# N-HANS/N-HANS

Measured on AMD Instinct MI355X. Metric: denoised audio seconds per second (16 kHz), whole job, higher is better.
Workload: dtype f16x3 (split hi+lo f16 operands, f32 accumulate); 1 GPU; 256 x 10 s 16 kHz synthetic mixture(s) per GPU, denoiser model, STFT+embed+mask+iSTFT end-to-end; clips_per_gpu=256, distinct_clips_per_gpu=256, frames_per_gpu=255488, weights=synthetic seed 7, parallelism=clip-sharded x1

## Files before the change

include/nhans_hip.h:

```cpp
#ifndef NHANS_HIP_H
#define NHANS_HIP_H

#include <stddef.h>
#include <stdint.h>

#ifdef __cplusplus
extern "C" {
#endif

#define NHANS_ABI_VERSION 5

#define NHANS_DENOISER 0
#define NHANS_SEPARATOR 1

#define NHANS_OK 0
#define NHANS_EINVAL (-1)
#define NHANS_EHIP (-2)
#define NHANS_ENOMEM (-3)
#define NHANS_ESHORT (-4)

#define NHANS_STATUS_SATURATED 1

#define NHANS_NUM_ACTIVATIONS 25

// ... 43 lines not shown
                        int nclips, const float* ctx_a_wav_dev, const int64_t* ctx_a_offsets_host,
                        const float* ctx_b_wav_dev, const int64_t* ctx_b_offsets_host,
                        float* denoised_wav_dev, float* mixed_wav_dev, float* logmag_out_dev,
                        float* phase_out_dev, float* logits_out_dev, float* emb_out_dev, void* stream);

int nhans_debug_block_output(nhans_ctx* ctx, const float* logmag_dev, const int64_t* frame_offsets_host,
                             int nclips, const float* emb_a_dev, const float* emb_b_dev,
                             int64_t frame0, int nframes, int block, float* out_dev, void* stream);

int nhans_debug_activation(nhans_ctx* ctx, const float* logmag_dev, const int64_t* frame_offsets_host,
                           int nclips, const float* emb_a_dev, const float* emb_b_dev,
                           int64_t frame0, int nframes, int index, float* out_dev, void* stream);
int nhans_debug_tower_activation(nhans_ctx* ctx, const float* ctx_logmag_dev, int n, int index, float* out_dev,
                                 void* stream);

int nhans_take_status(nhans_ctx* ctx, int* flags_out, void* stream);

int nhans_debug_launch_probe(size_t dynamic_lds_bytes, void* stream);

int nhans_debug_mfma_ceiling(double seconds, void* stream, double* sustained_tflops, double* first_tflops,
                             int* launches);

int nhans_debug_row_classes(int H, int KH, int stride, int pt, int* out, int cap);

uint32_t nhans_crc32c(uint32_t crc, const void* data_host, size_t nbytes);

typedef struct nhans_online nhans_online;

int nhans_online_open(nhans_ctx* ctx, int nstreams, const float* ctx_a_wav_dev, const int64_t* ctx_a_offsets_host,
                      const float* ctx_b_wav_dev, const int64_t* ctx_b_offsets_host, int want_mixed, void* stream,
                      nhans_online** out);

int nhans_online_open_slots(nhans_ctx* ctx, int nslots, int want_mixed, void* stream, nhans_online** out);

int nhans_online_restart(nhans_online* obj, int slot);

int nhans_online_set_context(nhans_online* obj, int slot, const float* ctx_a_wav_dev, int64_t na,
                             const float* ctx_b_wav_dev, int64_t nb, void* stream, int64_t* first_frame_out);

int nhans_online_set_embeddings(nhans_online* obj, int slot, const float* emb_a_dev, const float* emb_b_dev,
                                void* stream, int64_t* first_frame_out);


int nhans_online_push(nhans_online* obj, const float* in_dev, const int64_t* in_offsets_host, const int* end_host,
                      float* den_out_dev, float* mixed_out_dev, const int64_t* out_offsets_host,
                      int64_t* out_counts_host, void* stream);
// ... 106 lines not shown
```

n-hans_amd/csrc/conv_epilogue.h:

```cpp
#pragma once
#include "nhans_kernels.h"
#include <cstddef>

namespace nhans {

typedef float f32x16 __attribute__((ext_vector_type(16)));
typedef float f32x4 __attribute__((ext_vector_type(4)));
typedef _Float16 f16x8 __attribute__((ext_vector_type(8)));
typedef _Float16 f16x4 __attribute__((ext_vector_type(4)));

template <int I, int NM, int ND> __device__ __forceinline__ void pin_reads_between_mfmas() {
    if constexpr (I < ND) {
        __builtin_amdgcn_sched_group_barrier(0x008, (I + 1) * NM / ND - I * NM / ND, 0);
        __builtin_amdgcn_sched_group_barrier(0x100, 1, 0);
        pin_reads_between_mfmas<I + 1, NM, ND>();
    }
}

template <int I, int NM, int ND> __device__ __forceinline__ void pin_reads_front_loaded() {
    if constexpr (I < ND) {
        __builtin_amdgcn_sched_group_barrier(0x008, 1, 0);
        __builtin_amdgcn_sched_group_barrier(0x100, 1, 0);
        pin_reads_front_loaded<I + 1, NM, ND>();
    } else if constexpr (NM > ND) {
// ... 31 lines not shown
    else asm("v_fma_mix_f32 %0, %1, 1.0, %2 op_sel:[1,0,1] op_sel_hi:[1,0,1]" : "=v"(d) : "v"(hi_pair), "v"(lo_pair));
    return d;
}

__device__ __forceinline__ float split_load(const float* base, size_t row_floats, int n) {
    const _Float16* p = reinterpret_cast<const _Float16*>(base + row_floats) + (n >> 5) * 64 + (n & 31);
    return (float)p[0] + (float)p[32];
}

template <typename T> __device__ __forceinline__ T conv_karg(size_t offset) {
    typedef const __attribute__((address_space(4))) char* kptr;
    return *reinterpret_cast<const __attribute__((address_space(4))) T*>((kptr)__builtin_amdgcn_kernarg_segment_ptr() + offset);
}
#define CONV_KARG(FIELD) ::nhans::conv_karg<decltype(::nhans::ConvArgs::FIELD)>(offsetof(::nhans::ConvArgs, FIELD))

template <int BMROWS, int BNCOLS> constexpr size_t conv_epilogue_lds_bytes() {
    return (size_t)BMROWS * (BNCOLS + 4) * sizeof(float) + (size_t)BMROWS * sizeof(int4);
}

struct EpiTile {
    int m0;
    int tw, th;
    int b, r0, c0;
    __device__ __forceinline__ int operator()(int p, const ConvArgs& a) const {
        if (tw <= 0) {
            const int m = m0 + p;
            return m < a.M ? m : -1;
        }
        const int r = p / tw, c = p - r * tw;
        if (r >= th || r0 + r >= a.Ho || c0 + c >= a.Wo) return -1;
        return (b * a.Ho + r0 + r) * a.Wo + c0 + c;
    }
};

template <int PREC, int IDM, int OUTS, int PP, int PASSES, int LDC>
__device__ __forceinline__ void conv_epilogue_sweep(const ConvArgs& a, const float* ct, const int4* rowinfo,
                                                    int prow, int c4, int n) {
    constexpr int GP = PASSES < 8 ? PASSES : 8;
    static_assert(PASSES % GP == 0, "pass grouping");
    const int f_tf = a.tf ? 1 : 0;
    const float* __restrict__ cbp = a.cb;
    const float* __restrict__ tfp = a.tf ? a.tf : a.zero;
    f32x4 wsv = {1.f, 1.f, 1.f, 1.f}, idwv = {0.f, 0.f, 0.f, 0.f};
    if constexpr (PREC == 1) wsv = *reinterpret_cast<const f32x4*>(a.ws + n) * CONV_KARG(in_scale);
    if constexpr (IDM != 0) idwv = *reinterpret_cast<const f32x4*>(a.idw + n) * CONV_KARG(id_scale);
    const int hoff = (n >> 5) * 64 + (n & 31);
    const float lo_clamp = a.relu ? 0.f : -3.0e38f;
    const float osc = CONV_KARG(out_scale), slim = CONV_KARG(sat_limit);
    bool sat = false;
#pragma unroll 1
// ... 156 lines not shown
        }
    };

    Epi8Raw<IDM> ra[GP], rb[GP];
    issue(0, ra);
#pragma unroll
    for (int g = 0; g < NG; g += 2) {
        if (g + 1 < NG) issue(g + 1, rb);
        finish(ra);
        if (kDev && es && g == 0) {
            asm volatile("s_waitcnt lgkmcnt(0)" ::: "memory");
            es[2] = (long long)__builtin_amdgcn_s_memtime();
        }
        if (g + 2 < NG) issue(g + 2, ra);
        if (g + 1 < NG) finish(rb);
    }
    int* const satp = CONV_KARG(sat);
    if (sat && satp) atomicOr(satp, kSatActivation);
}

template <int TM, int TN, int PREC, int NTHREADS, int BMROWS, int BNCOLS>
__device__ __forceinline__ void conv_epilogue(const ConvArgs& a, f32x16 (&acc)[TM][TN], float* smem, EpiTile tile,
                                              int row_base, int col_base, int n_tile0, int tid, int lane,
                                              long long* es = nullptr ) {
    constexpr int LDC = BNCOLS + 4;
    constexpr int C4 = BNCOLS / 4;
    constexpr int PP = NTHREADS / C4;
    constexpr int PASSES = BMROWS / PP;
    float* ct = smem;
    int4* rowinfo = reinterpret_cast<int4*>(smem + BMROWS * LDC);

#pragma unroll
    for (int i = 0; i < TM; ++i)
#pragma unroll
        for (int j = 0; j < TN; ++j)
#pragma unroll
            for (int g = 0; g < 4; ++g) {
                const f32x4 v = {acc[i][j][4 * g], acc[i][j][4 * g + 1], acc[i][j][4 * g + 2], acc[i][j][4 * g + 3]};
                *reinterpret_cast<f32x4*>(ct + (row_base + i * 32 + (lane & 31)) * LDC + col_base + j * 32 + 8 * g +
                                          4 * (lane >> 5)) = v;
            }
    if (tid < BMROWS) {
        const int mz = tile(tid, a);
        const int m = mz < 0 ? (tile.tw > 0 ? tile(0, a) : a.M - 1) : mz;
        const uint32_t b = fd_div((uint32_t)m, a.fdHoWo);
        const uint32_t rem = (uint32_t)m - b * a.fdHoWo.d;
        const uint32_t ho = fd_div(rem, a.fdWo);
        const uint32_t wo = rem - ho * a.fdWo.d;
        const int clip = a.img_clip ? a.img_clip[b] : 0;
        const uint32_t hov = ho + (uint32_t)a.oh0;
        const int remv = (int)(hov * a.fdWo.d + wo);
        const int mv = mz < 0 ? mz : (int)(b * (uint32_t)a.Ho_full * a.fdWo.d) + remv;
        int ids;
        if (a.id_mode == 2 && a.id_win.t) {
            const int h = (int)hov * a.idsh;
            ids = win_row_ok(a.id_win, (int)b, h) ? win_row(a.id_win, (int)b, h) * a.idW + (int)wo * a.idsw : kNoRow;
        } else {
            ids = (int)((b * a.idH + hov * a.idsh) * a.idW + wo * a.idsw);
        }
        rowinfo[tid] = make_int4(clip * a.cb_stride, remv * a.N, mv, ids);
    }
    if (kDev && es) { asm volatile("s_waitcnt lgkmcnt(0)" ::: "memory"); es[0] = (long long)__builtin_amdgcn_s_memtime(); }
    __syncthreads();
    if (kDev && es) es[1] = (long long)__builtin_amdgcn_s_memtime();

    const int c4 = tid % C4, prow = tid / C4;
    const int n = n_tile0 + c4 * 4;
    const int f_tf = a.tf ? 1 : 0;
    const bool id_split = a.id_mode == 1 && a.id_split;
    const float* __restrict__ cbp = a.cb;
    const float* __restrict__ tfp = a.tf ? a.tf : a.zero;
    const bool vec = (a.Nreal == a.N) && !a.aux && (a.out_split || (a.ldo & 3) == 0) &&
                     (a.id_mode != 1 || id_split || (a.id_ld & 3) == 0);
// ... 55 lines not shown
```

n-hans_amd/csrc/conv_igemm_halo.hip:

```cpp
#include "conv_epilogue.h"
#include <cstdlib>

namespace nhans {

namespace {
constexpr int NCW = 8;
constexpr int NPW = 4;

template <int HBM_> struct HaloShape {
    static constexpr int HBM = HBM_;
    static constexpr int HR = HBM_ == 512 ? 544 : 320;
    static constexpr int BST = HBM_ == 512 ? 3 : 4;
    static constexpr int WN = HBM_ == 512 ? 1 : 2;
    static constexpr int NAP = HR * 8 / (NPW * 64);
};

template <int N> __device__ __forceinline__ void halo_wait_vmcnt() {
    asm volatile("s_waitcnt vmcnt(%0)" ::"n"(N) : "memory");
}
}

template <int BN, int PREC, int HBM_ = 256, int DBG = 0, int ABL = 0, int PWM = 0>
__global__ void __launch_bounds__((NCW + NPW) * 64) conv_igemm_halo(const ConvArgs a) {
    using SH = HaloShape<HBM_>;
    constexpr int HBM = SH::HBM, HR = SH::HR, BST = SH::BST, WN = SH::WN, NAP = SH::NAP;
    constexpr int PFD = BST - 1;
    constexpr int TM = 2;
    constexpr int TN = BN / (32 * WN);
    static_assert(HBM == (NCW / WN) * TM * 32 && BN == WN * TN * 32, "wave grid");
    static_assert(!PWM || (HBM == 256 && BST == 4), "pointwise mode: 256-pixel tiles, four weight stages");
    constexpr int A_BUF = (PWM ? HBM : HR) * 32;
    constexpr int NABUF = PWM ? 3 : 2;
    constexpr int NAPW = PWM ? HBM * 8 / (NPW * 64) : NAP;
    constexpr int B_STAGE = 32 * BN;
    constexpr int B_BASE = NABUF * A_BUF;
    constexpr int GBP = B_STAGE / 4 / (NPW * 64);
    extern __shared__ __attribute__((aligned(16))) float smem[];

    const int tid = threadIdx.x, lane = tid & 63;
    const int wave = __builtin_amdgcn_readfirstlane(tid >> 6);
    long long dbg_entry = 0;
    if constexpr (DBG) dbg_entry = (long long)__builtin_amdgcn_s_memtime();

    const int ntn = a.N / BN;
    int L;
    {
        const int nblk = gridDim.x, bid = blockIdx.x;
        const int q = nblk >> 3, r = nblk & 7, xcd = bid & 7, idx = bid >> 3;
        L = (xcd < r ? xcd * (q + 1) : r * (q + 1) + (xcd - r) * q) + idx;
    }
    const int mt = L / ntn, nt = L - mt * ntn;
    const int m0 = mt * HBM;
    const int nt0 = nt * (BN / 32);

    const int Wo = (int)a.fdWo.d;
    const int R0 = (int)fd_div((uint32_t)m0, a.fdWo);
    const int w0 = m0 - R0 * Wo;

    const int nseg = a.nseg;
    const int KW0 = a.seg[0].KW, KH0 = a.seg[0].KH, CC0 = a.seg[0].C >> 5;
    const int KH1 = nseg > 1 ? a.seg[1].KH : 0, CC1 = nseg > 1 ? (a.seg[1].C >> 5) : 0;
    const int nsup0 = KH0 * CC0 * (PWM ? KW0 : 1);
    const int nsup = nsup0 + KH1 * CC1;
    const int ntap0 = PWM ? nsup0 : nsup0 * KW0;
    const int total = ntap0 + KH1 * CC1;

    int segC = 0, kwC = 0, bufC = 0, supC = 0;
#define NH_NEXT_TAP()                                                                              \
    if constexpr (PWM) {                                                                           \
        bufC = bufC == NABUF - 1 ? 0 : bufC + 1;                                                   \
    } else if (++kwC >= (segC ? 1 : KW0)) {                                                        \
        kwC = 0;                                                                                   \
        bufC ^= 1;                                                                                 \
        if (++supC == nsup0) segC = 1;                                                             \
    }

    if (wave >= NCW) {
        const int pw = wave - NCW, ptid = tid - NCW * 64;
        if constexpr (!(ABL & 64)) __builtin_amdgcn_s_setprio(3);
        const int slot = lane & 7;
        const int nrows_all = a.M / Wo;
        const size_t bstride = (size_t)(a.N / 32) * 1024;
        constexpr unsigned kOob = 0x80000000u;
        const int b0 = (int)fd_div((uint32_t)m0, a.fdHoWo);
        int poff[NAPW], hov[NAPW], wiv[PWM ? NAPW : 1];
        int sH = 0, sW = 0, sC = 0;
        __amdgpu_buffer_rsrc_t srsrc;
#define NH_MAP_SEGMENT(S)                                                                          \
    {                                                                                              \
        const ConvSeg& g = a.seg[S];                                                               \
        sH = g.H; sW = g.W; sC = g.C;                                                              \
        {                                                                                          \
            const size_t fb_ = (size_t)g.H * g.W * g.C * 4;                                        \
            const size_t left_ = (size_t)(a.M / (a.Ho * Wo) - b0) * fb_;                           \
            srsrc = __builtin_amdgcn_make_buffer_rsrc(const_cast<float*>(g.src) + (size_t)b0 * (fb_ / 4), 0, \
                                                      (int)(left_ < 0x7FFFFFFFu ? left_ : 0x7FFFFFFFu), 0x00020000); \
        }                                                                                          \
        _Pragma("unroll") for (int d = 0; d < NAPW; ++d) {                                         \
            const int j = d * 32 + pw * 8 + (lane >> 3);                                           \
            const int sp = (slot ^ ((j >> 1) & 7)) * 4;                                            \
            int Rg, wi;                                                                            \
            bool ok;                                                                               \
            if (!PWM && g.KW > 1) {                                                                \
                const int n0 = Wo - w0 + g.KW - 1;                                                 \
                int i = 0, cj = w0 + j;                                                            \
                if (j >= n0) {                                                                     \
                    const int jj = j - n0;                                                         \
                    const int q = (int)fd_div((uint32_t)jj, a.fdWP);                               \
                    i = 1 + q;                                                                     \
                    cj = jj - q * (int)a.fdWP.d;                                                   \
                }                                                                                  \
                wi = cj - g.pl;                                                                    \
                Rg = R0 + i;                                                                       \
                ok = Rg < nrows_all && (unsigned)wi < (unsigned)g.W;                               \
            } else {                                                                               \
                const int m = m0 + j;                                                              \
                ok = j < HBM && m < a.M;                                                           \
                Rg = (int)fd_div((uint32_t)(ok ? m : 0), a.fdWo);                                  \
                wi = ((ok ? m : 0) - Rg * Wo) * g.sw - g.pl;                                       \
            }                                                                                      \
            if (!ok) { Rg = 0; wi = 0; }                                                           \
            const int b = (int)fd_div((uint32_t)(Rg * Wo), a.fdHoWo);                              \
            const int hi0 = (Rg - b * a.Ho) * g.sh - g.pt;                                         \
            poff[d] = ((((b - b0) * g.H + hi0) * g.W + wi) * g.C + sp) * 4;      \
            hov[d] = ok ? hi0 : -(1 << 28);                                                        \
            if constexpr (PWM) wiv[d] = wi;               \
        }                                                                                          \
    }
#define NH_GLDS(SRC, DST)                                                                          \
    __builtin_amdgcn_global_load_lds((const __attribute__((address_space(1))) void*)(SRC),        \
                                     (__attribute__((address_space(3))) void*)(DST), 16, 0, 0);

        int segA = 0, khA = 0, ccA = 0, supA = 0, kwA = 0;
#define NH_ISSUE_A(BUF)                                                                            \
    {                                                                                              \
        const int khoff_ = (khA * sW + (PWM ? kwA : 0)) * sC + ccA * 32;                           \
        const bool live_ = supA < nsup;                                                            \
        float* sa_ = smem + (BUF) * A_BUF + pw * 8 * 32;                                           \
        _Pragma("unroll") for (int d = 0; d < NAPW; ++d) {                                         \
            bool in_ = !(ABL & 1) && live_ && (unsigned)(hov[d] + khA) < (unsigned)sH;             \
            if constexpr (PWM) in_ = in_ && (unsigned)(wiv[d] + kwA) < (unsigned)sW;               \
            if constexpr (!(ABL & 2))                                                              \
                __builtin_amdgcn_raw_ptr_buffer_load_lds(srsrc, (__attribute__((address_space(3))) void*)(sa_ + d * 32 * 32), 16, \
                                                         in_ ? (unsigned)(poff[d] + khoff_ * 4) : kOob, 0, 0, 0); \
        }                                                                                          \
        ++supA;                                                                                    \
        if (PWM && ++kwA < KW0) {                  \
        } else if (kwA = 0, ++khA >= (segA ? KH1 : KH0)) {  \
            khA = 0;                                                                               \
            if (++ccA >= (segA ? CC1 : CC0)) {                                                     \
                ccA = 0;                                                                           \
                if (segA == 0 && nseg > 1) {                                                       \
                    segA = 1;                                                                      \
                    NH_MAP_SEGMENT(1)                                                              \
                }                                                                                  \
            }                                                                                      \
        }                                                                                          \
    }
        int tapB = 0;
        const __amdgpu_buffer_rsrc_t wr0 = __builtin_amdgcn_make_buffer_rsrc(const_cast<float*>(a.seg[0].wpk) + (size_t)nt0 * 1024, 0, 0x7FFFFFFF, 0x00020000);
        const __amdgpu_buffer_rsrc_t wr1 = __builtin_amdgcn_make_buffer_rsrc(const_cast<float*>(nseg > 1 ? a.seg[1].wpk : a.seg[0].wpk) + (size_t)nt0 * 1024, 0, 0x7FFFFFFF, 0x00020000);
        const unsigned wvo = (unsigned)ptid * 16u;
        const int bstride_b = (int)(bstride * 4);
        int wper = KH0 * KW0, wskip = (a.seg[0].KHfull - KH0) * KW0, wrun = 0;
        int wtap = a.seg[0].kh0 * KW0 - 1, wseg = 0;
#define NH_ISSUE_B(ST)                                                                             \
    {                                                                                              \
        if (tapB < total && !(ABL & 4)) {                                                          \
            if (tapB == ntap0) {                                                                   \
                wseg = 1; wtap = a.seg[1].kh0 * a.seg[1].KW; wrun = 1;                             \
                wper = KH1 * a.seg[1].KW; wskip = (a.seg[1].KHfull - KH1) * a.seg[1].KW;           \
            } else {                                                                               \
                if (wrun == wper) { wrun = 0; wtap += wskip; }                                     \
                ++wtap; ++wrun;                                                                    \
            }                                                                                      \
        }                                                                                          \
        ++tapB;                                                                                    \
        float* sb_ = smem + B_BASE + (ST) * B_STAGE;                                               \
        const int so_ = (ABL & 4) ? 0 : wtap * bstride_b;                                          \
        _Pragma("unroll") for (int j = 0; j < GBP; ++j)                                            \
            if constexpr (!(ABL & 8))                                                              \
                __builtin_amdgcn_raw_ptr_buffer_load_lds((wseg || (ABL & 4)) ? wr1 : wr0,          \
                    (__attribute__((address_space(3))) void*)(sb_ + (j * (NPW * 64) + pw * 64) * 4), 16, wvo, so_ + j * (NPW * 64) * 16, 0, 0); \
    }

        NH_MAP_SEGMENT(0)
        NH_ISSUE_A(0)
        NH_ISSUE_B(0)
// ... 162 lines not shown
            }
            acc[0][0][0] += k_;
        }
        __builtin_amdgcn_sched_barrier(0);
    }
    asm volatile("s_waitcnt lgkmcnt(0)" ::: "memory");
    __builtin_amdgcn_s_barrier();
    if constexpr (DBG) {
        if (a.dbg && lane == 0) {
            long long* d = a.dbg + ((size_t)blockIdx.x * (NCW + NPW) + wave) * 4;
            d[0] = (long long)__builtin_amdgcn_s_memtime() - dbg_t0; d[1] = dbg_t0 - dbg_entry; d[2] = 0; d[3] = dbg_bar;
        }
    }
#undef NH_READ_HALF
#undef NH_MFMA_HALF
#undef NH_NEXT_TAP
#undef NH_PIN_INTERLEAVE

    long long dbg_epi = 0;
    long long es[3] = {0, 0, 0};
    if constexpr (DBG) dbg_epi = (long long)__builtin_amdgcn_s_memtime();
    static_assert(conv_epilogue_lds_bytes<HBM, BN>() <= (size_t)(NABUF * A_BUF + BST * B_STAGE) * sizeof(float), "epilogue LDS");
    conv_epilogue<TM, TN, PREC, NCW * 64, HBM, BN>(a, acc, smem, EpiTile{m0, 0, 0, 0, 0, 0}, wm * 64, wn * TN * 32, nt * BN, tid, lane,
                                                   DBG ? es : nullptr);
    if constexpr (DBG) {
        const long long t_issued = (long long)__builtin_amdgcn_s_memtime();
        asm volatile("s_waitcnt vmcnt(0)" ::: "memory");
        if (a.dbg && lane == 0) {
            const long long t_end = (long long)__builtin_amdgcn_s_memtime();
            a.dbg[((size_t)blockIdx.x * (NCW + NPW) + wave) * 4 + 2] = t_end - dbg_epi;
            long long* e = a.dbg + (size_t)(4 << 20) + ((size_t)blockIdx.x * (NCW + NPW) + wave) * 8;
            e[0] = es[0] - dbg_epi; e[1] = es[1] - dbg_epi; e[2] = es[2] - dbg_epi; e[3] = t_issued - dbg_epi; e[4] = t_end - dbg_epi;
        }
    }
}

template <int BN, int PREC, int HBM_ = 256, int DBG = 0, int ABL = 0, int PWM = 0> static void launch_halo_t(const ConvArgs& a, hipStream_t s) {
    using SH = HaloShape<HBM_>;
    constexpr size_t lds = (size_t)((PWM ? 3 * SH::HBM : 2 * SH::HR) * 32 + SH::BST * 32 * BN) * sizeof(float);
    static_assert(lds <= 160 * 1024, "LDS of a gfx950 CU");
    static unsigned long long attr_devices = 0;
    set_max_dynamic_lds(reinterpret_cast<const void*>(&conv_igemm_halo<BN, PREC, HBM_, DBG, ABL, PWM>), lds, &attr_devices, "conv_igemm_halo");
    const int mtiles = (a.M + SH::HBM - 1) / SH::HBM;
    const int grid = mtiles * (a.N / BN);
    NHANS_LAUNCH("conv_igemm_halo", (conv_igemm_halo<BN, PREC, HBM_, DBG, ABL, PWM>), dim3(grid), dim3((NCW + NPW) * 64), lds, s, a);
}

static int halo_tile_pixels(const ConvArgs& a) { return (a.N % 128 != 0 && a.halo64_tile512) ? 512 : 256; }

bool conv_igemm_halo_eligible(const ConvArgs& a) {
    const ConvSeg& g = a.seg[0];
    if (g.KW < 3 || g.sw != 1 || a.Wo != g.W || g.pl < 0 || g.pl >= g.KW) return false;
    if (a.nseg > 1 && a.seg[1].KW != 1) return false;
    if (a.nseg > 2 || a.M % a.Wo != 0) return false;
    for (int i = 0; i < a.nseg; ++i) {
        const ConvSeg& q = a.seg[i];
        const double elems = (double)(a.M / (a.Ho * a.Wo)) * q.H * q.W * q.C;
        if (elems + 65536.0 >= 2147483648.0) return false;
    }
    const int hbm = halo_tile_pixels(a);
    const int nrows = (a.Wo - 1 + hbm - 1) / a.Wo + 1;
    return hbm + (g.KW - 1) * nrows <= (hbm == 512 ? HaloShape<512>::HR : HaloShape<256>::HR);
}

bool conv_igemm_halo_pw_eligible(const ConvArgs& a) {
    const ConvSeg& g = a.seg[0];
    if (a.nseg != 1 || a.N % 128 != 0 || a.kgroup != 0 || g.C % 32 != 0) return false;
// ... 61 lines not shown
```

n-hans_amd/csrc/host_ctx.hip:

```cpp
#include "host_internal.h"

namespace {

thread_local std::string g_err;

constexpr uint32_t kBlobVersion = 2;
struct BlobHeader {
    char magic[8];
    uint32_t version;
    uint32_t n_entries;
    uint64_t total_bytes;
};
struct BlobEntry {
    char name[48];
    uint64_t offset;
    uint64_t nfloats;
};

std::vector<BlockGeo> tower_geometry() {
    const int kh[4] = {8, 8, 4, 4}, kw[4] = {4, 4, 4, 4}, sh[4] = {3, 3, 1, 1}, sw[4] = {2, 2, 1, 2};
    const int co[4] = {64, 128, 256, 512};
    std::vector<BlockGeo> v;
    int h = kCtxFrames, w = kBins, c = 1;
    for (int i = 0; i < 4; ++i) {
// ... 343 lines not shown
    }
    else if (k == "conv_variant") {
        if (value < -1 || value > 2) return fail(NHANS_EINVAL, "conv_variant must be -1 (auto), 0, 1 or 2");
        c->conv_variant = (int)value;
    }
    else if (k == "calibrate") {
        if (value < 0 || value > 3) return fail(NHANS_EINVAL, "calibrate must be 1 (start), 0 (stop, set), 2 (stop, raise only) or 3 (stop, discard)");
        int rc = check_ctx(c); if (rc) return rc;
        if (value == 1) {
            HIP_TRY(hipDeviceSynchronize());
            HIP_TRY(hipMemset(c->amax_dev, 0, kNumAct * sizeof(unsigned)));
            c->calibrating = true;
        } else {
            if (!c->calibrating) return fail(NHANS_EINVAL, "calibrate: no bracket is open");
            if (value == 3) { c->calibrating = false; return NHANS_OK; }
            return finish_calibration(c, value == 2);
        }
    }
    else if (k == "winograd") c->wino = value != 0;
    else if (k == "winograd_f32_tensors") c->wino_f32 = (value == 2 || value == 3) ? (int)value : value != 0;
    else if (k == "split_k") c->split_k = value != 0;
    else if (k == "stream_1x1") c->stream_1x1 = value != 0;
    else if (k == "row_split") {
        if (value < 0 || value > 2) return fail(NHANS_EINVAL, "row_split must be 0, 1 or 2 (2: every conv that can be split, a measurement value)");
        c->row_split = (int)value;
    }
    else if (k == "precision") {
        if (value != 0 && value != 1) return fail(NHANS_EINVAL, "precision must be 0 (f32) or 1 (f16x3)");
        if (value == 1 && !c->A("head.dense.wpk_h"))
            return fail(NHANS_EINVAL, "the folded blob carries no split-f16 weights");
        c->prec = (int)value;
    }
    else return fail(NHANS_EINVAL, "unknown option " + k);
    return NHANS_OK;
}

int nhans_set_activation_exponents(nhans_ctx* c, const int* e, int n) {
    if (!c || !e || n != kNumAct) return fail(NHANS_EINVAL, "activation exponents: need NHANS_NUM_ACTIVATIONS values");
    for (int i = 0; i < n; ++i)
        if (e[i] < -60 || e[i] > 60) return fail(NHANS_EINVAL, "activation exponent outside [-60, 60]");
    std::copy(e, e + n, c->act_exp);
    tie_exponents(c);
    return NHANS_OK;
}

int nhans_get_activation_exponents(nhans_ctx* c, int* e_out, int n) {
    if (!c || !e_out || n != kNumAct) return fail(NHANS_EINVAL, "activation exponents: need NHANS_NUM_ACTIVATIONS values");
// ... 105 lines not shown
```

n-hans_amd/csrc/host_internal.h:

```cpp
#pragma once
#include "../../include/nhans_hip.h"
#include "nhans_kernels.h"

#include <algorithm>
#include <cmath>
#include <cstdio>
#include <cstdlib>
#include <cstring>
#include <limits>
#include <map>
#include <string>
#include <vector>

using namespace nhans;

#pragma GCC visibility push(hidden)

int fail(int code, const std::string& msg);

#define HIP_TRY(expr)                                                                          \
    do {                                                                                       \
        hipError_t e_ = (expr);                                                                \
        if (e_ != hipSuccess)                                                                  \
            return fail(NHANS_EHIP, std::string(#expr) + ": " + hipGetErrorString(e_));        \
// ... 18 lines not shown
#pragma GCC visibility pop

struct StackPlan {
    bool wino[8][3] = {};
};

struct nhans_ctx {
    int kind = 0, device = 0;
    StackPlan last_plan;
    float* blob_dev = nullptr;
    size_t blob_bytes = 0;
    std::map<std::string, const float*> arr;
    std::map<std::string, size_t> arr_n;
    std::vector<BlockGeo> tower, stack;
    int cond_cols = 0;
    std::vector<int> cond_off;
    char* ws = nullptr;
    size_t ws_bytes = 0, ws_top = 0;
    float* kscratch = nullptr;
    size_t kscratch_bytes = 0;
    static constexpr size_t kscratch_cap = (size_t)384 << 20;
    bool kscratch_failed = false;
    int stream_1x1 = 1;
    int row_split = 1;
    int split_k = 1;
    int* kcounter = nullptr;
    int kcounter_n = 1024;
    int64_t frames_per_chunk = 3776;
    int contexts_per_chunk = 64;
    int lookahead = kCenter;
    char* pin = nullptr;
    size_t pin_bytes = (size_t)16 << 20, pin_top = 0;
    bool profile = false;
    std::map<std::string, ProfEntry> prof;
    std::vector<hipEvent_t> event_pool;

    int prec = 0;
    int conv_variant = -1;
    int epi8 = 1;
    int ilv = 1;
    int wino = 1;
    int wino_f32 = 1;
    long long* dbg = nullptr;
    int* status_dev = nullptr;
    std::map<std::pair<int, int>, float*> rs_tab;
    int act_exp[kNumAct] = {};
    float act_amax[kNumAct] = {};
// ... 221 lines not shown
```

n-hans_amd/csrc/host_net.hip:

```cpp
#include "host_internal.h"

namespace {

void same_pad(int n, int k, int s, int* out, int* before) {
    *out = (n + s - 1) / s;
    int total = std::max((*out - 1) * s + k - n, 0);
    *before = total / 2;
}

void fill_epilogue_defaults(nhans_ctx* c, ConvArgs& a) {
    a.zero = c->A("zero");
    a.sat = c->status_dev;
    a.img_clip = nullptr; a.tf = nullptr; a.tt = nullptr; a.ff = nullptr; a.id_mode = 0; a.id = nullptr; a.id_ld = 0;
    a.idw = nullptr; a.idH = a.idW = 0; a.idsh = a.idsw = 1; a.relu = 1; a.aux = nullptr; a.aux_ld = 0;
    a.cb_stride = 0;
    a.prec = c->prec; a.out_split = c->prec; a.id_split = 0; a.ws = nullptr;
    a.in_scale = a.id_scale = a.out_scale = 1.f;
    a.sat_limit = kSatLimitF16;
    a.variant = c->conv_variant >= 0 ? c->conv_variant : (c->prec == 1 ? 2 : 0);
    a.dbg = kDev ? c->dbg : nullptr;
    a.epi8 = c->epi8;
    a.ilv = c->ilv;
    a.wino = c->wino; a.wino_u = nullptr; a.wino_ws = nullptr;
    a.kscratch = c->kscratch; a.kscratch_bytes = c->kscratch_bytes; a.kcounter = c->kcounter; a.kcounter_n = c->kcounter_n; a.kgroup = 0;
// ... 19 lines not shown
}

const char* run_conv(nhans_ctx* c, const ConvArgs& a0, hipStream_t s) {
    ConvArgs a = a0;
    if (kDev) {
        static const bool no_tf = [] { const char* e = getenv("NHANS_ABLATE_TF"); return e && atoi(e) != 0; }();
        if (no_tf) { a.tf = nullptr; a.tt = nullptr; a.ff = nullptr; }
    }
    if (a.kgroup < 0) {
        const size_t need = c->split_k ? conv_splitk_scratch_bytes(a) : 0;
        if (need > c->kscratch_bytes && need <= nhans_ctx::kscratch_cap && !c->kscratch_failed) {
            if (c->kscratch) { (void)hipFree(c->kscratch); c->kscratch = nullptr; c->kscratch_bytes = 0; }
            const size_t want = std::min(nhans_ctx::kscratch_cap, std::max(need, (size_t)32 << 20));
            if (hipMalloc(reinterpret_cast<void**>(&c->kscratch), want) == hipSuccess) c->kscratch_bytes = want;
            else { (void)hipGetLastError(); c->kscratch = nullptr; c->kscratch_failed = true; }
        }
        a.kscratch = c->split_k ? c->kscratch : nullptr;
        a.kscratch_bytes = c->kscratch_bytes;
    }
    Prof p(c, s, nullptr);
    const char* name = "conv_igemm";
    double mfma = 0;
    double fl = launch_conv_igemm(a, s, &name, &mfma);
    if (a.Ho_full != a.Ho) {
        double kfull = 0;
        for (int i = 0; i < a.nseg; ++i) kfull += (double)a.seg[i].KHfull * a.seg[i].KW * a.seg[i].C;
        fl = 2.0 * (double)a.M * kfull * (double)a.Nreal;
    }
    p.done(fl, 0, name, mfma);
    return name;
}

struct RowClass { int oh0, rows, kh0, kh; };

int row_classes(int H, int KH, int s, int pt, RowClass* out, int cap) {
    const int Ho = (H + s - 1) / s;
    int n = 0;
    for (int ho = 0; ho < Ho; ++ho) {
        const int hi0 = ho * s - pt;
        const int lo = std::max(0, -hi0), hi = std::min(KH, H - hi0);
        if (hi <= lo) return 0;
        if (n && out[n - 1].kh0 == lo && out[n - 1].kh == hi - lo) { ++out[n - 1].rows; continue; }
        if (n == cap) return -1;
        out[n++] = RowClass{ho, 1, lo, hi - lo};
    }
    return n;
}

bool row_split_pays(const ConvSeg& g, const RowClass* rc, int n) {
    int applied = 0, rows = 0;
    for (int i = 0; i < n; ++i) { applied += rc[i].rows * rc[i].kh; rows += rc[i].rows; }
    return 100 * (rows * g.KH - applied) >= 7 * rows * g.KH;
}

constexpr int kMaxRowClasses = 8;
bool halo_family(ConvArgs a) {
    if (a.variant < 2 || a.kgroup != 0 || a.N % 128 != 0 || a.in_f32 || conv_wino_eligible(a)) return false;
    a.halo64_tile512 = 0;
    return conv_igemm_halo_eligible(a) || conv_igemm_halo_pw_eligible(a);
}
bool run_conv_row_classes(nhans_ctx* c, const ConvArgs& a, hipStream_t s) {
    const ConvSeg& g = a.seg[0];
    if (!c->row_split || a.prec != 1 || a.Ho_full != a.Ho || a.M % (a.Ho * a.Wo) != 0 || !halo_family(a)) return false;
    if (a.nseg > 1 && a.seg[1].KH != 1) return false;
    RowClass rc[kMaxRowClasses];
    const int n = row_classes(g.H, g.KH, g.sh, g.pt, rc, kMaxRowClasses);
    if (n < 2 || (g.H + g.sh - 1) / g.sh != a.Ho) return false;
    if (c->row_split == 1 && !row_split_pays(g, rc, n)) return false;
    const int B = a.M / (a.Ho * a.Wo);
    ConvArgs q[kMaxRowClasses];
    for (int i = 0; i < n; ++i) {
        q[i] = a;
        q[i].Ho = rc[i].rows; q[i].M = B * rc[i].rows * a.Wo; q[i].oh0 = rc[i].oh0; q[i].Ho_full = a.Ho;
        q[i].fdHoWo = make_fastdiv((uint32_t)(rc[i].rows * a.Wo));
        ConvSeg& h = q[i].seg[0];
        h.KH = rc[i].kh; h.kh0 = rc[i].kh0; h.KHfull = g.KH; h.pt = g.pt - rc[i].kh0 - rc[i].oh0 * g.sh;
        h.nchunks = h.KH * h.KW * h.C / 32;
        if (a.nseg > 1) {
            ConvSeg& t = q[i].seg[1];
            if ((rc[i].oh0 + rc[i].rows - 1) * t.sh - t.pt >= t.H || rc[i].oh0 * t.sh - t.pt < 0) return false;
            t.pt -= rc[i].oh0 * t.sh;
        }
        q[i].wino_u = nullptr; q[i].wino_ws = nullptr;
        if (!halo_family(q[i])) return false;
    }
    for (int i = 0; i < n && !launch_error_pending(); ++i)
        if (std::strncmp(run_conv(c, q[i], s), "conv_igemm_halo", 15) != 0)
            note_refusal("row-class conv launch on a kernel that does not walk filter-row classes");
    return true;
}

bool wino_form(const ConvArgs& a) { return a.variant >= 2 && a.kgroup >= 0 && conv_wino_eligible(a); }
float sat_limit_for(const StackPlan& p, int b, int cv) { return b >= 0 && b < 8 && p.wino[b][cv] ? kSatLimitWinoInput : kSatLimitF16; }

bool stored_f32(const nhans_ctx* c, const StackPlan& p, int b, int cv) {
    if (c->prec != 1 || !c->wino_f32 || b < 0 || b > 7) return false;
    if (c->wino_f32 == 2) return b < 4 && !(b == 3 && cv == 1);
    if (c->wino_f32 == 3) return b == 1 && cv == 1;
    if (cv == 0) return p.wino[b][2] && (b == 0 || p.wino[b][1]);
    if (b == 7) return false;
    const BlockGeo& nx = c->stack[b + 1];
    return p.wino[b][2] && p.wino[b + 1][1] && nx.cin == nx.cout && p.wino[b + 1][2];
}

void tap(nhans_ctx* c, int idx, const float* buf, size_t words, int chan, hipStream_t s, bool f32_layout = false) {
    if (c->calibrating) launch_absmax(buf, words, c->prec && !f32_layout, c->up(idx), c->amax_dev + idx, s);
    if (c->cap_idx != idx) return;
// ... 500 lines not shown
    rc = h2d(c, sb.foff_dev, foff, (nclips + 1) * sizeof(int64_t), s); if (rc) return rc;
    launch_frame_index(sb.foff_dev, nclips, total, c->lookahead, sb.f_clip, sb.f_t, sb.f_T, s);
    launch_cond(ea, eb, nclips, c->A("cond.w"), c->A("cond.base"), c->cond_cols, sb.cb_all, s);
    const float* res = run_stack_chunk(c, logmag, nullptr, sb, frame0, nframes, block + 1, s);
    size_t per;
    if (block == 8) per = (size_t)26 * 512;
    else per = (size_t)c->stack[block].hout * c->stack[block].wout * c->stack[block].cout;
    if (c->prec && block < 8 && stored_f32(c, c->last_plan, block, 1)) launch_scale_copy(res, per * nframes, c->up(SA(block, 1)), out, s);
    else if (c->prec) launch_unsplit(res, (int64_t)nframes * (int64_t)(per / (block == 8 ? 512 : c->stack[block].cout)),
                                block == 8 ? 512 : c->stack[block].cout, c->up(block == 8 ? kActHead : SA(block, 1)), out, s);
    else HIP_TRY(hipMemcpyAsync(out, res, per * nframes * 4, hipMemcpyDeviceToDevice, s));
    return NHANS_OK;
}

int nhans_debug_row_classes(int H, int KH, int stride, int pt, int* out, int cap) {
    if (H < 1 || KH < 1 || stride < 1 || pt < 0 || cap < 0 || (cap && !out)) return fail(NHANS_EINVAL, "row classes: bad argument");
    std::vector<RowClass> rc((size_t)(H + stride - 1) / stride);
    const int n = row_classes(H, KH, stride, pt, rc.data(), (int)rc.size());
    if (n > cap) return fail(NHANS_EINVAL, "row classes: " + std::to_string(n) + " classes, room for " + std::to_string(cap));
    for (int i = 0; i < n; ++i) { out[4 * i] = rc[i].oh0; out[4 * i + 1] = rc[i].rows; out[4 * i + 2] = rc[i].kh0; out[4 * i + 3] = rc[i].kh; }
    return n;
}

int nhans_debug_block_output(nhans_ctx* c, const float* logmag, const int64_t* foff, int nclips, const float* ea,
                             const float* eb, int64_t frame0, int nframes, int block, float* out, void* stream) {
    Call call(c, stream);
    if (call.rc) return call.rc;
    return call.finish(debug_block_output_body(c, logmag, foff, nclips, ea, eb, frame0, nframes, block, out, stream));
}

static int debug_activation_body(nhans_ctx* c, const float* logmag, const int64_t* foff, int nclips, const float* ea,
                                 const float* eb, int64_t frame0, int nframes, int index, float* out, void* stream) {
    int rc = NHANS_OK;
    if (!logmag || !foff || !ea || !eb || !out || nclips < 1 || nframes < 1) return fail(NHANS_EINVAL, "bad argument");
    if (index < SA(0, 0) || index >= kNumAct)
        return fail(NHANS_EINVAL, "activation index outside the stack's 8 .. " + std::to_string(kNumAct - 1) + " (tower tensors: nhans_debug_tower_activation)");
    hipStream_t s = static_cast<hipStream_t>(stream);
    const int64_t total = foff[nclips];
    if (frame0 < 0 || frame0 + nframes > total) return fail(NHANS_EINVAL, "frame range outside batch");
    const int64_t wf = std::min<int64_t>(c->frames_per_chunk, nframes);
    rc = ws_reserve(c, stack_ws_bytes(c, total, nclips, wf)); if (rc) return rc;
    StackBufs sb;
    stack_take(c, total, nclips, wf, &sb);
    rc = h2d(c, sb.foff_dev, foff, (nclips + 1) * sizeof(int64_t), s); if (rc) return rc;
    launch_frame_index(sb.foff_dev, nclips, total, c->lookahead, sb.f_clip, sb.f_t, sb.f_T, s);
    launch_cond(ea, eb, nclips, c->A("cond.w"), c->A("cond.base"), c->cond_cols, sb.cb_all, s);
// ... 69 lines not shown
```

n-hans_amd/csrc/nhans_kernels.h:

```cpp
#pragma once
#include <hip/hip_runtime.h>
#include <stdint.h>

#include <tuple>
#include <utility>
#include <vector>

namespace nhans {

constexpr int kWin = 400, kHop = 160, kBins = 201, kMixWin = 35, kCtxFrames = 200, kEmb = 512;
constexpr int kCenter = kMixWin / 2;
constexpr int64_t kMaxFramesPerChunk = ((int64_t)1 << 31) / ((int64_t)kMixWin * kBins * 64);

#ifdef NHANS_DEV
constexpr bool kDev = true;
int dev_ablate();
#else
constexpr bool kDev = false;
constexpr int dev_ablate() { return 0; }
#endif

void note_launch(const char* kernel, hipError_t launch_rc);
bool launch_error_pending();
void note_refusal(const char* what);
// ... 36 lines not shown
struct WinRows {
    const int* t;
    const int* T;
    int row0, pad;
    const int* rb;
};
constexpr int kNoRow = -2147483647 - 1;
__device__ __forceinline__ bool win_row_ok(const WinRows& w, int b, int h) {
    return (unsigned)(w.t[b] + h - w.pad) < (unsigned)w.T[b];
}
__device__ __forceinline__ int win_row(const WinRows& w, int b, int h) {
    return (w.rb ? w.rb[b] : w.row0 + b) + h;
}

struct ConvSeg {
    const float* src;
    const float* wpk;
    int H, W, C;
    int KH, KW, sh, sw, pt, pl;
    int nchunks;
    int kh0, KHfull;
};

struct ConvArgs {
    ConvSeg seg[2];
    int nseg;
    int Ho, Wo;
    int M;
    int oh0, Ho_full;
    int N;
    int Nreal;
    int ldo;
    float* out;
    const float* cb;
    int cb_stride;
    const int* img_clip;
    const float* tf;
    const float* tt;
    const float* ff;
    int id_mode;
    const float* id;
    int id_ld;
    const float* idw;
    int idH, idW, idsh, idsw;
    WinRows id_win;
    int relu;
    float* aux;
    int aux_ld;
    const float* zero;
    int prec;
    int out_split;
    int id_split;
// ... 163 lines not shown
```

n-hans_amd/hip.py:

```python
import ctypes
import json
import os
import sys

_HERE = os.path.dirname(os.path.abspath(__file__))
LIB_PATH = os.environ.get("NHANS_LIB") or os.path.join(_HERE, "csrc", "libnhans_hip.so")

DENOISER, SEPARATOR = 0, 1
KIND_CODE = {"denoiser": DENOISER, "separator": SEPARATOR}

_int, _i64, _dbl, _vp = ctypes.c_int, ctypes.c_int64, ctypes.c_double, ctypes.c_void_p
_size, _str = ctypes.c_size_t, ctypes.c_char_p
_ip, _i64p, _vpp = ctypes.POINTER(_int), ctypes.POINTER(_i64), ctypes.POINTER(_vp)
_fp, _dp = ctypes.POINTER(ctypes.c_float), ctypes.POINTER(_dbl)
SIGNATURES = {
    "nhans_abi_version": (_int, []),
    "nhans_last_error": (_str, []),
    "nhans_num_frames": (_i64, [_i64]),
    "nhans_create": (_int, [_int, _vp, _size, _int, _vpp]),
    "nhans_create_ex": (_int, [_int, _vp, _size, _int, _ip, _int, _vpp]),
    "nhans_destroy": (None, [_vp]),
    "nhans_set_option": (_int, [_vp, _str, _i64]),
    "nhans_set_activation_exponents": (_int, [_vp, _ip, _int]),
    "nhans_get_activation_exponents": (_int, [_vp, _ip, _int]),
    "nhans_get_activation_amax": (_int, [_vp, _fp, _int]),
    "nhans_workspace_bytes": (_size, [_vp, _i64, _int]),
    "nhans_stft_features": (_int, [_vp, _vp, _i64p, _int, _int, _vp, _vp, _vp]),
    "nhans_embed": (_int, [_vp, _vp, _int, _vp, _vp]),
    "nhans_mask_net": (_int, [_vp, _vp, _i64p, _int, _vp, _vp, _vp, _vp, _vp]),
    "nhans_istft": (_int, [_vp, _vp, _vp, _i64p, _int, _i64p, _vp, _vp]),
    "nhans_enhance_clips": (_int, [_vp, _vp, _i64p, _int, _vp, _i64p, _vp, _i64p, _vp, _vp, _vp, _vp, _vp, _vp, _vp]),
    "nhans_debug_block_output": (_int, [_vp, _vp, _i64p, _int, _vp, _vp, _i64, _int, _int, _vp, _vp]),
    "nhans_debug_activation": (_int, [_vp, _vp, _i64p, _int, _vp, _vp, _i64, _int, _int, _vp, _vp]),
    "nhans_debug_tower_activation": (_int, [_vp, _vp, _int, _int, _vp, _vp]),
    "nhans_take_status": (_int, [_vp, _ip, _vp]),
    "nhans_debug_launch_probe": (_int, [_size, _vp]),
    "nhans_debug_mfma_ceiling": (_int, [_dbl, _vp, _dp, _dp, _ip]),
    "nhans_debug_row_classes": (_int, [_int, _int, _int, _int, _ip, _int]),
    "nhans_crc32c": (ctypes.c_uint32, [ctypes.c_uint32, _vp, _size]),
    "nhans_online_open": (_int, [_vp, _int, _vp, _i64p, _vp, _i64p, _int, _vp, _vpp]),
    "nhans_online_open_slots": (_int, [_vp, _int, _int, _vp, _vpp]),
    "nhans_online_restart": (_int, [_vp, _int]),
    "nhans_online_set_context": (_int, [_vp, _int, _vp, _i64, _vp, _i64, _vp, _i64p]),
    "nhans_online_set_embeddings": (_int, [_vp, _int, _vp, _vp, _vp, _i64p]),
    "nhans_online_push": (_int, [_vp, _vp, _i64p, _ip, _vp, _vp, _i64p, _i64p, _vp]),
    "nhans_online_out_counts": (_int, [_vp, _i64p, _ip, _i64p]),
    "nhans_online_rewind": (_int, [_vp]),
    "nhans_online_set_lookahead": (_int, [_vp, _int, _int]),
    "nhans_online_close": (None, [_vp]),
    "nhans_resample_out_count": (_i64, [_i64, _int, _int]),
    "nhans_resample_emitted": (_i64, [_i64, _int, _int, _int]),
    "nhans_resample_taps": (_int, [_int, _int, _dp, _int]),
    "nhans_resample": (_int, [_vp, _vp, _int, _i64p, _int, _int, _int, _int, _vp, _i64p, _vp]),
    "nhans_peak_normalise": (_int, [_vp, _vp, _i64p, _int, _int, _vp, _vp]),
    "nhans_channel_mean": (_int, [_vp, _vp, _int, _i64, _vp, _vp]),
    "nhans_resampler_open": (_int, [_vp, _int, _int, _int, _int, _int, _vpp]),
    "nhans_resampler_set_peak": (_int, [_vp, _dbl]),
    "nhans_resampler_push": (_int, [_vp, _vp, _i64p, _ip, _vp, _i64p, _i64p, _vp]),
    "nhans_resampler_out_counts": (_int, [_vp, _i64p, _ip, _i64p]),
    "nhans_resampler_restart": (_int, [_vp, _int]),
    "nhans_resampler_close": (None, [_vp]),
# ... 102 lines not shown
```

Measured before the change: 512.7 audio-seconds/s.

## Launch row-split halo convolutions as one grid over filter-row classes

Row-split convolutions, where boundary output rows use a truncated filter height, now run as a single halo-conv launch instead of one launch per row class. A per-class table (up to three classes, ordered by descending filter rows) is carried in ConvArgs, and each workgroup picks its class from its block index. This aims to remove per-class launch overhead and the tail underutilisation of small class grids. In exchange, kernel arguments grow and the kernel does extra class lookups. The default row_split becomes the new one-grid mode, and a debug entry point reports the grid layout.

```diff
diff --git a/include/nhans_hip.h b/include/nhans_hip.h
--- a/include/nhans_hip.h
+++ b/include/nhans_hip.h
@@ -89,6 +89,8 @@
                              int* launches);
 
 int nhans_debug_row_classes(int H, int KH, int stride, int pt, int* out, int cap);
+
+int nhans_debug_row_grid(int H, int KH, int stride, int pt, int Wo, int64_t frames, int tile, int* out, int cap);
 
 uint32_t nhans_crc32c(uint32_t crc, const void* data_host, size_t nbytes);
 
diff --git a/n-hans_amd/csrc/conv_epilogue.h b/n-hans_amd/csrc/conv_epilogue.h
--- a/n-hans_amd/csrc/conv_epilogue.h
+++ b/n-hans_amd/csrc/conv_epilogue.h
@@ -77,10 +77,11 @@
     int m0;
     int tw, th;
     int b, r0, c0;
-    __device__ __forceinline__ int operator()(int p, const ConvArgs& a) const {
+    __device__ __forceinline__ int operator()(int p, const ConvArgs& a) const { return (*this)(p, a, a.M); }
+    __device__ __forceinline__ int operator()(int p, const ConvArgs& a, int M) const {
         if (tw <= 0) {
             const int m = m0 + p;
-            return m < a.M ? m : -1;
+            return m < M ? m : -1;
         }
         const int r = p / tw, c = p - r * tw;
         if (r >= th || r0 + r >= a.Ho || c0 + c >= a.Wo) return -1;
@@ -283,7 +284,8 @@
 template <int TM, int TN, int PREC, int NTHREADS, int BMROWS, int BNCOLS>
 __device__ __forceinline__ void conv_epilogue(const ConvArgs& a, f32x16 (&acc)[TM][TN], float* smem, EpiTile tile,
                                               int row_base, int col_base, int n_tile0, int tid, int lane,
-                                              long long* es = nullptr ) {
+                                              long long* es = nullptr ,
+                                              const ConvRowClass* rc = nullptr ) {
     constexpr int LDC = BNCOLS + 4;
     constexpr int C4 = BNCOLS / 4;
     constexpr int PP = NTHREADS / C4;
@@ -302,14 +304,16 @@
                                           4 * (lane >> 5)) = v;
             }
     if (tid < BMROWS) {
-        const int mz = tile(tid, a);
-        const int m = mz < 0 ? (tile.tw > 0 ? tile(0, a) : a.M - 1) : mz;
-        const uint32_t b = fd_div((uint32_t)m, a.fdHoWo);
-        const uint32_t rem = (uint32_t)m - b * a.fdHoWo.d;
+        const int vM = rc ? rc->M : a.M;
+        const FastDiv& fdv = rc ? rc->fdHoWo : a.fdHoWo;
+        const int mz = tile(tid, a, vM);
+        const int m = mz < 0 ? (tile.tw > 0 ? tile(0, a) : vM - 1) : mz;
+        const uint32_t b = fd_div((uint32_t)m, fdv);
+        const uint32_t rem = (uint32_t)m - b * fdv.d;
         const uint32_t ho = fd_div(rem, a.fdWo);
         const uint32_t wo = rem - ho * a.fdWo.d;
         const int clip = a.img_clip ? a.img_clip[b] : 0;
-        const uint32_t hov = ho + (uint32_t)a.oh0;
+        const uint32_t hov = ho + (uint32_t)(rc ? rc->oh0 : a.oh0);
         const int remv = (int)(hov * a.fdWo.d + wo);
         const int mv = mz < 0 ? mz : (int)(b * (uint32_t)a.Ho_full * a.fdWo.d) + remv;
         int ids;
diff --git a/n-hans_amd/csrc/conv_igemm_halo.hip b/n-hans_amd/csrc/conv_igemm_halo.hip
--- a/n-hans_amd/csrc/conv_igemm_halo.hip
+++ b/n-hans_amd/csrc/conv_igemm_halo.hip
@@ -43,10 +43,12 @@
     if constexpr (DBG) dbg_entry = (long long)__builtin_amdgcn_s_memtime();
 
     const int ntn = a.N / BN;
+    const int bid = blockIdx.x;
+    const ConvRowClass& rc = a.cls[(bid >= a.cls[1].wg0 ? 1 : 0) + (bid >= a.cls[2].wg0 ? 1 : 0)];
     int L;
     {
-        const int nblk = gridDim.x, bid = blockIdx.x;
-        const int q = nblk >> 3, r = nblk & 7, xcd = bid & 7, idx = bid >> 3;
+        const int nblk = rc.nwg, l = bid - rc.wg0;
+        const int q = nblk >> 3, r = nblk & 7, xcd = l & 7, idx = l >> 3;
         L = (xcd < r ? xcd * (q + 1) : r * (q + 1) + (xcd - r) * q) + idx;
     }
     const int mt = L / ntn, nt = L - mt * ntn;
@@ -58,7 +60,7 @@
     const int w0 = m0 - R0 * Wo;
 
     const int nseg = a.nseg;
-    const int KW0 = a.seg[0].KW, KH0 = a.seg[0].KH, CC0 = a.seg[0].C >> 5;
+    const int KW0 = a.seg[0].KW, KH0 = rc.KH, CC0 = a.seg[0].C >> 5;
     const int KH1 = nseg > 1 ? a.seg[1].KH : 0, CC1 = nseg > 1 ? (a.seg[1].C >> 5) : 0;
     const int nsup0 = KH0 * CC0 * (PWM ? KW0 : 1);
     const int nsup = nsup0 + KH1 * CC1;
@@ -79,10 +81,10 @@
         const int pw = wave - NCW, ptid = tid - NCW * 64;
         if constexpr (!(ABL & 64)) __builtin_amdgcn_s_setprio(3);
         const int slot = lane & 7;
-        const int nrows_all = a.M / Wo;
+        const int nrows_all = rc.M / Wo;
         const size_t bstride = (size_t)(a.N / 32) * 1024;
         constexpr unsigned kOob = 0x80000000u;
-        const int b0 = (int)fd_div((uint32_t)m0, a.fdHoWo);
+        const int b0 = (int)fd_div((uint32_t)m0, rc.fdHoWo);
         int poff[NAPW], hov[NAPW], wiv[PWM ? NAPW : 1];
         int sH = 0, sW = 0, sC = 0;
         __amdgpu_buffer_rsrc_t srsrc;
@@ -115,13 +117,13 @@
                 ok = Rg < nrows_all && (unsigned)wi < (unsigned)g.W;                               \
             } else {                                                                               \
                 const int m = m0 + j;                                                              \
-                ok = j < HBM && m < a.M;                                                           \
+                ok = j < HBM && m < rc.M;                                                          \
                 Rg = (int)fd_div((uint32_t)(ok ? m : 0), a.fdWo);                                  \
                 wi = ((ok ? m : 0) - Rg * Wo) * g.sw - g.pl;                                       \
             }                                                                                      \
             if (!ok) { Rg = 0; wi = 0; }                                                           \
-            const int b = (int)fd_div((uint32_t)(Rg * Wo), a.fdHoWo);                              \
-            const int hi0 = (Rg - b * a.Ho) * g.sh - g.pt;                                         \
+            const int b = (int)fd_div((uint32_t)(Rg * Wo), rc.fdHoWo);                             \
+            const int hi0 = (Rg - b * rc.Ho) * g.sh - ((S) ? rc.pt1 : rc.pt);                      \
             poff[d] = ((((b - b0) * g.H + hi0) * g.W + wi) * g.C + sp) * 4;      \
             hov[d] = ok ? hi0 : -(1 << 28);                                                        \
             if constexpr (PWM) wiv[d] = wi;               \
@@ -163,7 +165,7 @@
         const unsigned wvo = (unsigned)ptid * 16u;
         const int bstride_b = (int)(bstride * 4);
         int wper = KH0 * KW0, wskip = (a.seg[0].KHfull - KH0) * KW0, wrun = 0;
-        int wtap = a.seg[0].kh0 * KW0 - 1, wseg = 0;
+        int wtap = rc.kh0 * KW0 - 1, wseg = 0;
 #define NH_ISSUE_B(ST)                                                                             \
     {                                                                                              \
         if (tapB < total && !(ABL & 4)) {                                                          \
@@ -372,7 +374,7 @@
     if constexpr (DBG) dbg_epi = (long long)__builtin_amdgcn_s_memtime();
     static_assert(conv_epilogue_lds_bytes<HBM, BN>() <= (size_t)(NABUF * A_BUF + BST * B_STAGE) * sizeof(float), "epilogue LDS");
     conv_epilogue<TM, TN, PREC, NCW * 64, HBM, BN>(a, acc, smem, EpiTile{m0, 0, 0, 0, 0, 0}, wm * 64, wn * TN * 32, nt * BN, tid, lane,
-                                                   DBG ? es : nullptr);
+                                                   DBG ? es : nullptr, &rc);
     if constexpr (DBG) {
         const long long t_issued = (long long)__builtin_amdgcn_s_memtime();
         asm volatile("s_waitcnt vmcnt(0)" ::: "memory");
@@ -385,14 +387,26 @@
     }
 }
 
-template <int BN, int PREC, int HBM_ = 256, int DBG = 0, int ABL = 0, int PWM = 0> static void launch_halo_t(const ConvArgs& a, hipStream_t s) {
+template <int BN, int PREC, int HBM_ = 256, int DBG = 0, int ABL = 0, int PWM = 0> static void launch_halo_t(const ConvArgs& a0, hipStream_t s) {
     using SH = HaloShape<HBM_>;
+    ConvArgs a = a0;
+    if (a.ncls < 0 || a.ncls > kMaxGridClasses) { note_refusal("conv_igemm_halo (row-class table)"); return; }
+    if (a.ncls == 0) {
+        a.ncls = 1;
+        a.cls[0] = ConvRowClass{0, 0, 0, a.Ho, a.M, a.oh0, a.fdHoWo, a.seg[0].KH, a.seg[0].kh0, a.seg[0].pt, a.seg[0].nchunks, a.nseg > 1 ? a.seg[1].pt : 0};
+    }
+    const int mtiles = conv_row_class_tiles(a.cls, a.ncls, SH::HBM), ntn = a.N / BN;
+    if ((double)mtiles * ntn >= 2147483648.0) { note_refusal("conv_igemm_halo (grid)"); return; }
+    for (int i = 0; i < a.ncls; ++i) {
+        a.cls[i].wg0 = a.cls[i].tile0 * ntn;
+        a.cls[i].nwg = ((i + 1 < a.ncls ? a.cls[i + 1].tile0 : mtiles) - a.cls[i].tile0) * ntn;
+    }
+    for (int i = a.ncls; i < kMaxGridClasses; ++i) { a.cls[i] = ConvRowClass{}; a.cls[i].tile0 = a.cls[i].wg0 = 0x7FFFFFFF; }
     constexpr size_t lds = (size_t)((PWM ? 3 * SH::HBM : 2 * SH::HR) * 32 + SH::BST * 32 * BN) * sizeof(float);
     static_assert(lds <= 160 * 1024, "LDS of a gfx950 CU");
     static unsigned long long attr_devices = 0;
     set_max_dynamic_lds(reinterpret_cast<const void*>(&conv_igemm_halo<BN, PREC, HBM_, DBG, ABL, PWM>), lds, &attr_devices, "conv_igemm_halo");
-    const int mtiles = (a.M + SH::HBM - 1) / SH::HBM;
-    const int grid = mtiles * (a.N / BN);
+    const int grid = mtiles * ntn;
     NHANS_LAUNCH("conv_igemm_halo", (conv_igemm_halo<BN, PREC, HBM_, DBG, ABL, PWM>), dim3(grid), dim3((NCW + NPW) * 64), lds, s, a);
 }
 
diff --git a/n-hans_amd/csrc/host_ctx.hip b/n-hans_amd/csrc/host_ctx.hip
--- a/n-hans_amd/csrc/host_ctx.hip
+++ b/n-hans_amd/csrc/host_ctx.hip
@@ -389,7 +389,8 @@
     else if (k == "split_k") c->split_k = value != 0;
     else if (k == "stream_1x1") c->stream_1x1 = value != 0;
     else if (k == "row_split") {
-        if (value < 0 || value > 2) return fail(NHANS_EINVAL, "row_split must be 0, 1 or 2 (2: every conv that can be split, a measurement value)");
+        if (value < 0 || value > 4)
+            return fail(NHANS_EINVAL, "row_split must be 0 .. 4 (1: class launches, 3: one grid per split conv; 2 / 4: of every conv that can be split, measurement values)");
         c->row_split = (int)value;
     }
     else if (k == "precision") {
diff --git a/n-hans_amd/csrc/host_internal.h b/n-hans_amd/csrc/host_internal.h
--- a/n-hans_amd/csrc/host_internal.h
+++ b/n-hans_amd/csrc/host_internal.h
@@ -64,7 +64,7 @@
     static constexpr size_t kscratch_cap = (size_t)384 << 20;
     bool kscratch_failed = false;
     int stream_1x1 = 1;
-    int row_split = 1;
+    int row_split = 3;
     int split_k = 1;
     int* kcounter = nullptr;
     int kcounter_n = 1024;
diff --git a/n-hans_amd/csrc/host_net.hip b/n-hans_amd/csrc/host_net.hip
--- a/n-hans_amd/csrc/host_net.hip
+++ b/n-hans_amd/csrc/host_net.hip
@@ -65,7 +65,11 @@
     const char* name = "conv_igemm";
     double mfma = 0;
     double fl = launch_conv_igemm(a, s, &name, &mfma);
-    if (a.Ho_full != a.Ho) {
+    if (a.ncls > 1) {
+        double mk = 0;
+        for (int i = 0; i < a.ncls; ++i) mk += (double)a.cls[i].M * (a.cls[i].nchunks + (a.nseg > 1 ? a.seg[1].nchunks : 0)) * 32.0;
+        mfma = 3.0 * 2.0 * mk * (double)a.N;
+    } else if (a.Ho_full != a.Ho) {
         double kfull = 0;
         for (int i = 0; i < a.nseg; ++i) kfull += (double)a.seg[i].KHfull * a.seg[i].KW * a.seg[i].C;
         fl = 2.0 * (double)a.M * kfull * (double)a.Nreal;
@@ -90,10 +94,16 @@
     return n;
 }
 
-bool row_split_pays(const ConvSeg& g, const RowClass* rc, int n) {
+constexpr int kSplitPercentLaunches = 7, kSplitPercentGrid = 7;
+bool row_split_pays(const ConvSeg& g, const RowClass* rc, int n, bool one_grid) {
     int applied = 0, rows = 0;
     for (int i = 0; i < n; ++i) { applied += rc[i].rows * rc[i].kh; rows += rc[i].rows; }
-    return 100 * (rows * g.KH - applied) >= 7 * rows * g.KH;
+    return 100 * (rows * g.KH - applied) >= (one_grid ? kSplitPercentGrid : kSplitPercentLaunches) * rows * g.KH;
+}
+
+void row_grid_order(const RowClass* rc, int n, int* order) {
+    for (int i = 0; i < n; ++i) order[i] = i;
+    std::stable_sort(order, order + n, [&](int x, int y) { return rc[x].kh > rc[y].kh; });
 }
 
 constexpr int kMaxRowClasses = 8;
@@ -109,7 +119,9 @@
     RowClass rc[kMaxRowClasses];
     const int n = row_classes(g.H, g.KH, g.sh, g.pt, rc, kMaxRowClasses);
     if (n < 2 || (g.H + g.sh - 1) / g.sh != a.Ho) return false;
-    if (c->row_split == 1 && !row_split_pays(g, rc, n)) return false;
+    bool grid = c->row_split >= 3 && n <= kMaxGridClasses;
+    if (c->row_split == 3 && !row_split_pays(g, rc, n, true)) grid = false;
+    if (!grid && (c->row_split == 1 || c->row_split == 3) && !row_split_pays(g, rc, n, false)) return false;
     const int B = a.M / (a.Ho * a.Wo);
     ConvArgs q[kMaxRowClasses];
     for (int i = 0; i < n; ++i) {
@@ -126,6 +138,23 @@
         }
         q[i].wino_u = nullptr; q[i].wino_ws = nullptr;
         if (!halo_family(q[i])) return false;
+    }
+    if (grid) {
+        const bool halo = conv_igemm_halo_eligible(a);
+        ConvArgs m = a;
+        int order[kMaxGridClasses];
+        row_grid_order(rc, n, order);
+        m.ncls = n;
+        for (int i = 0; i < n; ++i) {
+            const ConvArgs& k = q[order[i]];
+            if (conv_igemm_halo_eligible(k) != halo) return false;
+            m.cls[i] = ConvRowClass{0, 0, 0, k.Ho, k.M, k.oh0, k.fdHoWo, k.seg[0].KH, k.seg[0].kh0, k.seg[0].pt, k.seg[0].nchunks,
+                                    a.nseg > 1 ? k.seg[1].pt : 0};
+        }
+        m.wino_u = nullptr; m.wino_ws = nullptr;
+        if (std::strncmp(run_conv(c, m, s), "conv_igemm_halo", 15) != 0)
+            note_refusal("row-class conv launch on a kernel that does not walk filter-row classes");
+        return true;
     }
     for (int i = 0; i < n && !launch_error_pending(); ++i)
         if (std::strncmp(run_conv(c, q[i], s), "conv_igemm_halo", 15) != 0)
@@ -672,6 +701,29 @@
     return n;
 }
 
+int nhans_debug_row_grid(int H, int KH, int stride, int pt, int Wo, int64_t frames, int tile, int* out, int cap) {
+    if (H < 1 || KH < 1 || stride < 1 || pt < 0 || Wo < 1 || frames < 1 || tile < 1 || cap < 0 || (cap && !out))
+        return fail(NHANS_EINVAL, "row grid: bad argument");
+    const int Ho = (H + stride - 1) / stride;
+    if ((double)frames * Ho * Wo >= 2147483648.0) return fail(NHANS_EINVAL, "row grid: 2^31 output pixels or more");
+    RowClass rc[kMaxGridClasses];
+    const int n = row_classes(H, KH, stride, pt, rc, kMaxGridClasses);
+    if (n < 0) return fail(NHANS_EINVAL, "row grid: more than " + std::to_string(kMaxGridClasses) + " classes");
+    if (n > cap) return fail(NHANS_EINVAL, "row grid: " + std::to_string(n) + " classes, room for " + std::to_string(cap));
+    int order[kMaxGridClasses];
+    row_grid_order(rc, n, order);
+    ConvRowClass cls[kMaxGridClasses];
+    for (int i = 0; i < n; ++i) { cls[i] = ConvRowClass{}; cls[i].M = (int)(frames * rc[order[i]].rows * Wo); }
+    const int total = conv_row_class_tiles(cls, n, tile);
+    for (int i = 0; i < n; ++i) {
+        const RowClass& r = rc[order[i]];
+        const int next = i + 1 < n ? cls[i + 1].tile0 : total;
+        const int v[6] = {r.oh0, r.rows, r.kh0, r.kh, cls[i].tile0, next - cls[i].tile0};
+        std::copy(v, v + 6, out + 6 * i);
+    }
+    return n;
+}
+
 int nhans_debug_block_output(nhans_ctx* c, const float* logmag, const int64_t* foff, int nclips, const float* ea,
                              const float* eb, int64_t frame0, int nframes, int block, float* out, void* stream) {
     Call call(c, stream);
diff --git a/n-hans_amd/csrc/nhans_kernels.h b/n-hans_amd/csrc/nhans_kernels.h
--- a/n-hans_amd/csrc/nhans_kernels.h
+++ b/n-hans_amd/csrc/nhans_kernels.h
@@ -82,12 +82,29 @@
     int kh0, KHfull;
 };
 
+struct ConvRowClass {
+    int tile0;
+    int wg0, nwg;
+    int Ho, M, oh0;
+    FastDiv fdHoWo;
+    int KH, kh0, pt, nchunks;
+    int pt1;
+};
+constexpr int kMaxGridClasses = 3;
+inline int conv_row_class_tiles(ConvRowClass* cls, int n, int tile) {
+    int t = 0;
+    for (int i = 0; i < n; ++i) { cls[i].tile0 = t; t += (cls[i].M + tile - 1) / tile; }
+    return t;
+}
+
 struct ConvArgs {
     ConvSeg seg[2];
     int nseg;
     int Ho, Wo;
     int M;
     int oh0, Ho_full;
+    int ncls;
+    ConvRowClass cls[kMaxGridClasses];
     int N;
     int Nreal;
     int ldo;
diff --git a/n-hans_amd/hip.py b/n-hans_amd/hip.py
--- a/n-hans_amd/hip.py
+++ b/n-hans_amd/hip.py
@@ -37,6 +37,7 @@
     "nhans_debug_launch_probe": (_int, [_size, _vp]),
     "nhans_debug_mfma_ceiling": (_int, [_dbl, _vp, _dp, _dp, _ip]),
     "nhans_debug_row_classes": (_int, [_int, _int, _int, _int, _ip, _int]),
+    "nhans_debug_row_grid": (_int, [_int, _int, _int, _int, _int, _i64, _int, _ip, _int]),
     "nhans_crc32c": (ctypes.c_uint32, [ctypes.c_uint32, _vp, _size]),
     "nhans_online_open": (_int, [_vp, _int, _vp, _i64p, _vp, _i64p, _int, _vp, _vpp]),
     "nhans_online_open_slots": (_int, [_vp, _int, _int, _vp, _vpp]),
```

New measurement: 515.6 audio-seconds/s (median of 6 runs). No clear change (+0.6%).
